# chzhang18/RAG

Hardware: AMD Instinct MI355X
Metric: disparity maps/sec at 384x1248 D=192 (Matching-Net forward) (higher is better)
Workload: dtype f32 (RAGMI_F32X3: level-3/6/12 3x3x3 convolutions with fp32 operands split into power-of-two-scaled FP16 hi+lo halves on the 16-bit matrix cores, hi*hi + hi*lo + lo*hi, fp32 accumulate: fp32-class accuracy, bound in include/rag_amd.h; strict_fp32 holds the RAGMI_F32 number); 1 GPU; BASELINE configs[1]: 1 stereo pair(s)/GPU/step, 384x1248, D=192, f32, all-conv genotype, (left_fea,right_fea)->disp, inputs resident in HBM; global_batch=1, launch=hipGraph, ranks_seen=1

## Files before the change

### rag_amd/csrc/disp.hip

```cpp
#include "disp_common.h"

namespace ragmi {

struct DispArgs {
  const void* cost;
  float* out;
  DispGeom g;
};

struct DispMoments {
  float pv = 0.f, m1 = 0.f, m2 = 0.f, xs = 0.f, pk = 0.f;
  float b1[3] = {0.f, 0.f, 0.f}, b2[3] = {0.f, 0.f, 0.f};
  __device__ __forceinline__ void add_chain(int j, float e, float x, float fd) {
    const float t = fd - pv, et = e * t;
    b1[j] += et;
    b2[j] = fmaf(et, t, b2[j]);
    xs = fmaf(e, x, xs);
    pk = fmaxf(pk, e);
  }
  __device__ __forceinline__ void flush() {
    m1 += (b1[0] + b1[1]) + b1[2];
    m2 += (b2[0] + b2[1]) + b2[2];
    b1[0] = b1[1] = b1[2] = b2[0] = b2[1] = b2[2] = 0.f;
  }
  __device__ __forceinline__ void store(float* stats, int64_t b, int64_t npix, int64_t o, float s) const {
    const float c = m1 / s;
    float* const p = stats + b * 3 * npix + o;
    p[0] = fmaxf(fmaf(-c, c, m2 / s), 0.f);
    p[npix] = pk / s;
    p[2 * npix] = fmaxf(fmaf(-0.6931471805599453f, xs / s, logf(s)), 0.f);
  }
};

struct DispWindow {
  float ks = 0.f, rf = 0.f, w0 = 0.f, w1 = 0.f;
  float c0[3] = {0.f, 0.f, 0.f}, c1[3] = {0.f, 0.f, 0.f};
  __device__ __forceinline__ void add_chain(int j, float e, float fd) {
    const float t = fd - ks, ew = fabsf(t) <= rf ? e : 0.f;
    c0[j] += ew;
    c1[j] = fmaf(ew, t, c1[j]);
  }
  __device__ __forceinline__ void flush() {
    w0 += (c0[0] + c0[1]) + c0[2];
    w1 += (c1[0] + c1[1]) + c1[2];
    c0[0] = c0[1] = c0[2] = c1[0] = c1[1] = c1[2] = 0.f;
  }
  __device__ __forceinline__ void store(float* mode, int64_t b, int64_t npix, int64_t o, float s) const {
    float* const p = mode + b * 3 * npix + o;
    p[0] = ks;
    p[npix] = w0 > 0.f ? ks + w1 / w0 : ks;
    p[2 * npix] = w0 / s;
  }
};

template <class T, bool STATS, bool MODE>
__global__ __launch_bounds__(256) void disp_softargmin_kernel(DispArgs a, float* stats, float* mode, int radius) {
  static_assert(STATS || !MODE, "the mode instantiations write the statistics too");
  extern __shared__ float4 ztab[];
  const DispGeom& g = a.g;
  disp_fill_taps(ztab, g);
  __syncthreads();
  const int64_t npix = (int64_t)g.Ho * g.Wo;
  const int64_t o = (int64_t)blockIdx.x * 256 + threadIdx.x;
  if (o >= npix) return;
  const int b = blockIdx.y;
  const DispPlaneSampler<T> smp(static_cast<const T*>(a.cost) + (int64_t)b * g.d * (g.h * g.w), g, (int)(o / g.Wo), (int)(o % g.Wo));
  DispSoftmax sm;
  DispMoments mo;
  DispWalk walk(ztab, smp, g.d);
  for (int dd = 0; dd < g.maxdisp; ++dd) {
    const float t = walk.sample(dd);
    const DispSoftmax::Step k = sm.weigh(t);
    if constexpr (STATS) {
      if (k.up) {
        mo.flush();
        const float dl = (float)dd - mo.pv;
        mo.m2 = k.x * fmaf(dl, fmaf(dl, sm.s, -2.f * mo.m1), mo.m2);
        mo.m1 = k.x * fmaf(-dl, sm.s, mo.m1);
        mo.xs = sm.s > 0.f ? k.x * fmaf(k.xa, sm.s, mo.xs) : 0.f;
        mo.pv = (float)dd;
        mo.pk = 1.f;
      } else {
        mo.add_chain(0, k.x, k.xa, (float)dd);
      }
      if ((dd & 15) == 15) mo.flush();
    }
    sm.add(k, dd, t);
  }
  const float s = sm.s;
  a.out[(int64_t)b * npix + o] = sm.ws / s;
  if constexpr (STATS) {
    mo.flush();
    mo.store(stats, b, npix, o, s);
  }
  if constexpr (MODE) {
    DispWindow wd;
    wd.ks = mo.pv;
    wd.rf = (float)radius;
    const int ks = (int)mo.pv, d_lo = max(ks - radius, 0), d_hi = min(ks + radius, g.maxdisp - 1);
    DispWalk window(ztab, smp, g.d, (int)ztab[d_lo].x);
    for (int dd = d_lo; dd <= d_hi; ++dd) {
      wd.add_chain(0, __builtin_amdgcn_exp2f((window.sample(dd) - sm.m) * DISP_LOG2E), (float)dd);
      if (((dd - d_lo) & 15) == 15) wd.flush();
    }
    wd.flush();
    wd.store(mode, b, npix, o, s);
  }
}

constexpr int DX3_TY = 8, DX3_TX = 32, DX3_CR = 5, DX3_CC = 13, DX3_CP = DX3_CR * DX3_CC;

template <class T, bool STATS, bool MODE>
__global__ __launch_bounds__(256) void disp_softargmin_x3_kernel(DispArgs a, float* stats, float* mode, int radius) {
  static_assert(STATS || !MODE, "the mode instantiations write the statistics too");
  extern __shared__ __attribute__((aligned(16))) float dx3_lds[];
  const DispGeom& g = a.g;
  float4* const ztab = reinterpret_cast<float4*>(dx3_lds);
  float* const tile = dx3_lds + 4 * g.maxdisp;
  const int tid = threadIdx.x, tx = tid % DX3_TX, ty = tid / DX3_TX;
  const int ntx = (g.Wo + DX3_TX - 1) / DX3_TX, nty = (g.Ho + DX3_TY - 1) / DX3_TY, ntile = ntx * nty;
  const int chunk = (ntile + 7) / 8, jb = blockIdx.x;
  const int tidx = (jb & 7) * chunk + (jb >> 3);
  if ((jb >> 3) >= chunk || tidx >= ntile) return;
  const int ox0 = (tidx % ntx) * DX3_TX, oy0 = (tidx / ntx) * DX3_TY, b = blockIdx.z;
  const int ox = min(ox0 + tx, g.Wo - 1), oy = min(oy0 + ty, g.Ho - 1);
  const int cy0 = lin_index(oy0, g.h, g.Ho, g.sh, 0).i0, cx0 = lin_index(ox0, g.w, g.Wo, g.sw, 0).i0;
  const int hw = g.h * g.w, D = g.d;
  const T* base = static_cast<const T*>(a.cost) + (int64_t)b * D * hw;
  for (int i = tid; i < D * DX3_CP; i += 256) {
    const int z = i / DX3_CP, r = i % DX3_CP;
    const int gy = min(cy0 + r / DX3_CC, g.h - 1), gx = min(cx0 + r % DX3_CC, g.w - 1);
    tile[i] = ld(base + (int64_t)z * hw + gy * g.w + gx);
  }
  for (int dd = tid; dd < g.maxdisp; dd += 256) {
    const LinIdx lz = lin_index(dd, D, g.maxdisp, g.sd, 0);
    const int k = dd / 3;
    float4 e = make_float4(0.f, 0.f, 0.f, (float)dd);
    if (lz.i0 < k) { e.x = lz.w0; e.y = lz.w1; }
    else if (lz.i1 != lz.i0) { e.y = lz.w0; e.z = lz.w1; }
    else e.y = lz.w0 + lz.w1;
    ztab[dd] = e;
  }
  const LinIdx ly = lin_index(oy, g.h, g.Ho, g.sh, 0);
  const LinIdx lx = lin_index(ox, g.w, g.Wo, g.sw, 0);
  const float* const t00 = tile + (ly.i0 - cy0) * DX3_CC + (lx.i0 - cx0);
  const float* const t01 = t00 + (lx.i1 - lx.i0);
  const float* const t10 = t00 + (ly.i1 - ly.i0) * DX3_CC;
  const float* const t11 = t10 + (lx.i1 - lx.i0);
  __syncthreads();
  auto plane = [&](int z) {
    const int o = z * DX3_CP;
    return lerp2(ly.w0, lerp2(lx.w0, t00[o], lx.w1, t01[o]), ly.w1, lerp2(lx.w0, t10[o], lx.w1, t11[o]));
  };
  float s = 0.f, ws = 0.f;
  DispMoments mo;
  int am = 0;
  DispWindow wd;
  wd.rf = (float)radius;
  float lo = INFINITY;
  auto sample = [&](int j, const float4 tb, float vp, float vc, float vn) __attribute__((always_inline)) {
    const float c = fmaf(tb.x, vp, fmaf(tb.y, vc, tb.z * vn));
    const float x = (lo - c) * DISP_LOG2E;
    const float e = __builtin_amdgcn_exp2f(x);
    s += e;
    ws = fmaf(e, tb.w, ws);
    if constexpr (STATS) mo.add_chain(j, e, x, tb.w);
    if constexpr (MODE) wd.add_chain(j, e, tb.w);
  };
  auto fold = [&]() __attribute__((always_inline)) {
    if constexpr (STATS) mo.flush();
    if constexpr (MODE) wd.flush();
  };
  if (D == 64) {
    float v[64];
#pragma unroll
    for (int z = 0; z < 64; ++z) {
      v[z] = plane(z);
      lo = fminf(lo, v[z]);
      if ((z & 7) == 7) __builtin_amdgcn_sched_barrier(0);
    }
    if constexpr (STATS) {
#pragma unroll
      for (int z = 63; z >= 0; --z) am = v[z] == lo ? z : am;
      mo.pv = (float)(3 * am + 1);
      if constexpr (MODE) wd.ks = am == 0 ? 0.f : mo.pv;
      __builtin_amdgcn_sched_barrier(0);
    }
#pragma unroll
    for (int k = 0; k < 64; ++k) {
      const float vp_ = v[k > 0 ? k - 1 : 0], vc_ = v[k], vn_ = v[k < 63 ? k + 1 : 63];
#pragma unroll
      for (int j = 0; j < 3; ++j) sample(j, ztab[3 * k + j], vp_, vc_, vn_);
      if ((k & 7) == 7) {
        fold();
        __builtin_amdgcn_sched_barrier(0);
      }
    }
  } else {
#pragma clang loop unroll_count(4) vectorize(disable)
  for (int z = 0; z < D; ++z) {
    const float vz = plane(z);
    if constexpr (STATS) am = vz < lo ? z : am;
    lo = fminf(lo, vz);
  }
  if constexpr (STATS) mo.pv = (float)(3 * am + 1);
  if constexpr (MODE) wd.ks = am == 0 ? 0.f : mo.pv;
  float vc = plane(0), vp = vc, vn = plane(min(1, D - 1));
  for (int k = 0; k < D; ++k) {
#pragma unroll
    for (int j = 0; j < 3; ++j) sample(j, ztab[3 * k + j], vp, vc, vn);
    vp = vc; vc = vn; vn = plane(min(k + 2, D - 1));
    if ((k & 7) == 7) fold();
  }
  fold();
  }
  if (ox0 + tx < g.Wo && oy0 + ty < g.Ho) {
    a.out[(int64_t)b * g.Ho * g.Wo + (int64_t)oy * g.Wo + ox] = ws / s;
    if constexpr (STATS) mo.store(stats, b, (int64_t)g.Ho * g.Wo, (int64_t)oy * g.Wo + ox, s);
    if constexpr (MODE) wd.store(mode, b, (int64_t)g.Ho * g.Wo, (int64_t)oy * g.Wo + ox, s);
  }
}

template <class T, bool STATS, bool MODE>
__global__ __launch_bounds__(256) void disparity_regression_kernel(const T* __restrict__ prob, float* __restrict__ out, float* __restrict__ stats,
                                                                  float* __restrict__ mode, int D, int64_t hw, int radius) {
  static_assert(STATS || !MODE, "the mode instantiations write the statistics too");
  const int64_t o = (int64_t)blockIdx.x * 256 + threadIdx.x;
  if (o >= hw) return;
  const int b = blockIdx.y;
  const T* p = prob + (int64_t)b * D * hw + o;
  float acc = 0.f;
#pragma unroll 8
  for (int dd = 0; dd < D; ++dd) acc = fmaf(ld(p + (int64_t)dd * hw), (float)dd, acc);
  out[(int64_t)b * hw + o] = acc;
  if constexpr (STATS) {
    float var[8] = {0.f, 0.f, 0.f, 0.f, 0.f, 0.f, 0.f, 0.f}, ent[8] = {0.f, 0.f, 0.f, 0.f, 0.f, 0.f, 0.f, 0.f}, pk = 0.f;
    float best = -INFINITY;
    int ks = 0;
    for (int d0 = 0; d0 < D; d0 += 8) {
      static_for<8>([&](auto J) {
        constexpr int j = decltype(J)::value;
        if (d0 + j < D) {
          const float q = ld(p + (int64_t)(d0 + j) * hw), t = (float)(d0 + j) - acc;
          var[j] = fmaf(q * t, t, var[j]);
          ent[j] = q > 0.f ? fmaf(q, logf(q), ent[j]) : ent[j];
          pk = fmaxf(pk, q);
          if constexpr (MODE) {
            if (q > best) {
              best = q;
              ks = d0 + j;
            }
          }
        }
      });
    }
    float* const st = stats + (int64_t)b * 3 * hw + o;
    st[0] = ((var[0] + var[1]) + (var[2] + var[3])) + ((var[4] + var[5]) + (var[6] + var[7]));
    st[hw] = pk;
    st[2 * hw] = 0.f - (((ent[0] + ent[1]) + (ent[2] + ent[3])) + ((ent[4] + ent[5]) + (ent[6] + ent[7])));
    if constexpr (MODE) {
      float w0[8] = {0.f, 0.f, 0.f, 0.f, 0.f, 0.f, 0.f, 0.f}, w1[8] = {0.f, 0.f, 0.f, 0.f, 0.f, 0.f, 0.f, 0.f};
      const int d_lo = max(ks - radius, 0), d_hi = min(ks + radius, D - 1);
      for (int d0 = d_lo; d0 <= d_hi; d0 += 8) {
        static_for<8>([&](auto J) {
          constexpr int j = decltype(J)::value;
          if (d0 + j <= d_hi) {
            const float q = ld(p + (int64_t)(d0 + j) * hw);
            w0[j] += q;
            w1[j] = fmaf(q, (float)(d0 + j - ks), w1[j]);
          }
        });
      }
      const float m0 = ((w0[0] + w0[1]) + (w0[2] + w0[3])) + ((w0[4] + w0[5]) + (w0[6] + w0[7]));
      const float m1 = ((w1[0] + w1[1]) + (w1[2] + w1[3])) + ((w1[4] + w1[5]) + (w1[6] + w1[7]));
      float* const mp = mode + (int64_t)b * 3 * hw + o;
      mp[0] = (float)ks;
      mp[hw] = m0 != 0.f ? (float)ks + m1 / m0 : (float)ks;
      mp[2 * hw] = m0;
    }
  }
}

template <bool STATS, bool MODE>
int launch_disp_softargmin(const char* name, const void* cost, void* out, void* stats, void* mode, int B, int d, int h, int w,
                           int maxdisp, int Ho, int Wo, int radius, int dtype, void* stream) {
  RAGMI_REQUIRE(B > 0 && d > 0 && h > 0 && w > 0 && maxdisp > 0 && Ho > 0 && Wo > 0, RAGMI_EINVAL, "%s: non-positive size", name);
  if constexpr (MODE)
    RAGMI_REQUIRE(radius >= 0 && radius <= maxdisp, RAGMI_EINVAL, "%s: radius %d not in [0, maxdisp = %d]", name, radius, maxdisp);
  RAGMI_REQUIRE(dtype_ok(dtype), RAGMI_EUNSUPPORTED, "%s: dtype %d not built", name, dtype);
  RAGMI_REQUIRE(B <= 65535 && (int64_t)h * w < (1ll << 30), RAGMI_EUNSUPPORTED, "%s: size too large", name);
  const DispArgs a{cost, (float*)out, disp_geom(d, h, w, maxdisp, Ho, Wo)};
  const size_t lds = (size_t)maxdisp * sizeof(float4);
  RAGMI_REQUIRE(lds <= 64 * 1024, RAGMI_EUNSUPPORTED, "%s: maxdisp %d exceeds the tap table (4096)", name, maxdisp);
  const size_t lds3 = lds + (size_t)d * DX3_CP * sizeof(float);
  const bool tiled = maxdisp == 3 * d && Ho == 3 * h && Wo == 3 * w && lds3 <= 64 * 1024, bf16 = dtype == RAGMI_BF16;
  const dim3 grid((unsigned)ceil_div((int64_t)Ho * Wo, 256), B);
  const dim3 g3((unsigned)ceil_div(Wo, DX3_TX), (unsigned)ceil_div(Ho, DX3_TY), (unsigned)B);
  const dim3 g1((unsigned)(ceil_div((int64_t)g3.x * g3.y, 8) * 8), 1, (unsigned)B);
  void (*const kernel)(DispArgs, float*, float*, int) =
      tiled ? (bf16 ? disp_softargmin_x3_kernel<bf16_t, STATS, MODE> : disp_softargmin_x3_kernel<float, STATS, MODE>)
            : (bf16 ? disp_softargmin_kernel<bf16_t, STATS, MODE> : disp_softargmin_kernel<float, STATS, MODE>);
  hipLaunchKernelGGL(kernel, tiled ? g1 : grid, dim3(256), tiled ? lds3 : lds, static_cast<hipStream_t>(stream), a, (float*)stats,
                     (float*)mode, radius);
  return check_launch(name);
}

template <bool STATS, bool MODE>
int launch_disparity_regression(const char* name, const void* prob, void* out, void* stats, void* mode, int B, int D, int H, int W,
                                int radius, int dtype, void* stream) {
  RAGMI_REQUIRE(B > 0 && D > 0 && H > 0 && W > 0, RAGMI_EINVAL, "%s: non-positive size", name);
  if constexpr (MODE) RAGMI_REQUIRE(radius >= 0 && radius <= D, RAGMI_EINVAL, "%s: radius %d not in [0, D = %d]", name, radius, D);
  RAGMI_REQUIRE(dtype_ok(dtype), RAGMI_EUNSUPPORTED, "%s: dtype %d not built", name, dtype);
  RAGMI_REQUIRE(B <= 65535, RAGMI_EUNSUPPORTED, "%s: B too large", name);
  const int64_t hw = (int64_t)H * W;
  const dim3 grid((unsigned)ceil_div(hw, 256), B);
  const hipStream_t q = static_cast<hipStream_t>(stream);
  if (dtype == RAGMI_BF16)
    hipLaunchKernelGGL((disparity_regression_kernel<bf16_t, STATS, MODE>), grid, dim3(256), 0, q, (const bf16_t*)prob, (float*)out,
                       (float*)stats, (float*)mode, D, hw, radius);
  else
    hipLaunchKernelGGL((disparity_regression_kernel<float, STATS, MODE>), grid, dim3(256), 0, q, (const float*)prob, (float*)out,
                       (float*)stats, (float*)mode, D, hw, radius);
  return check_launch(name);
}

}

extern "C" int ragmi_disp_softargmin_fwd(const void* cost, void* out, int B, int d, int h, int w, int maxdisp, int Ho,
                                         int Wo, int dtype, void* stream) {
  RAGMI_REQUIRE(cost && out, RAGMI_EINVAL, "disp_softargmin: null pointer");
  return ragmi::launch_disp_softargmin<false, false>("disp_softargmin", cost, out, nullptr, nullptr, B, d, h, w, maxdisp, Ho, Wo, 0, dtype,
                                                     stream);
}
extern "C" int ragmi_disp_softargmin_stats_fwd(const void* cost, void* out, void* stats, int B, int d, int h, int w, int maxdisp,
                                               int Ho, int Wo, int dtype, void* stream) {
  RAGMI_REQUIRE(cost && out && stats, RAGMI_EINVAL, "disp_softargmin_stats: null pointer");
  return ragmi::launch_disp_softargmin<true, false>("disp_softargmin_stats", cost, out, stats, nullptr, B, d, h, w, maxdisp, Ho, Wo, 0,
                                                    dtype, stream);
}
extern "C" int ragmi_disp_softargmin_mode_fwd(const void* cost, void* out, void* stats, void* mode, int B, int d, int h, int w,
                                              int maxdisp, int Ho, int Wo, int radius, int dtype, void* stream) {
  RAGMI_REQUIRE(cost && out && stats && mode, RAGMI_EINVAL, "disp_softargmin_mode: null pointer");
  return ragmi::launch_disp_softargmin<true, true>("disp_softargmin_mode", cost, out, stats, mode, B, d, h, w, maxdisp, Ho, Wo, radius,
                                                   dtype, stream);
}

extern "C" int ragmi_disparity_regression_fwd(const void* prob, void* out, int B, int D, int H, int W, int dtype,
                                              void* stream) {
  RAGMI_REQUIRE(prob && out, RAGMI_EINVAL, "disparity_regression: null pointer");
  return ragmi::launch_disparity_regression<false, false>("disparity_regression", prob, out, nullptr, nullptr, B, D, H, W, 0, dtype, stream);
}
extern "C" int ragmi_disparity_regression_stats_fwd(const void* prob, void* out, void* stats, int B, int D, int H, int W, int dtype,
                                                    void* stream) {
  RAGMI_REQUIRE(prob && out && stats, RAGMI_EINVAL, "disparity_regression_stats: null pointer");
  return ragmi::launch_disparity_regression<true, false>("disparity_regression_stats", prob, out, stats, nullptr, B, D, H, W, 0, dtype,
                                                         stream);
}
extern "C" int ragmi_disparity_regression_mode_fwd(const void* prob, void* out, void* stats, void* mode, int B, int D, int H, int W,
                                                   int radius, int dtype, void* stream) {
  RAGMI_REQUIRE(prob && out && stats && mode, RAGMI_EINVAL, "disparity_regression_mode: null pointer");
  return ragmi::launch_disparity_regression<true, true>("disparity_regression_mode", prob, out, stats, mode, B, D, H, W, radius, dtype,
                                                        stream);
}
```

### rag_amd/csrc/disp_common.h

```cpp
#pragma once
#include "common.h"

namespace ragmi {

struct DispGeom {
  int d, h, w, maxdisp, Ho, Wo;
  float sd, sh, sw;
};
inline DispGeom disp_geom(int d, int h, int w, int maxdisp, int Ho, int Wo) {
  return DispGeom{d, h, w, maxdisp, Ho, Wo, lin_scale(d, maxdisp, 0), lin_scale(h, Ho, 0), lin_scale(w, Wo, 0)};
}

constexpr float DISP_LOG2E = 1.4426950408889634f;

__device__ __forceinline__ void disp_fill_taps(float4* ztab, const DispGeom& g) {
  for (int dd = threadIdx.x; dd < g.maxdisp; dd += 256) {
    const LinIdx lz = lin_index(dd, g.d, g.maxdisp, g.sd, 0);
    const bool same = lz.i1 == lz.i0;
    ztab[dd] = make_float4((float)lz.i0, lz.w0, same ? 0.f : lz.w1, same ? lz.w1 : 0.f);
  }
}

template <class T>
struct DispPlaneSampler {
  const T* base;
  int hw, o00, o01, o10, o11;
  float wy0, wy1, wx0, wx1;
  __device__ __forceinline__ DispPlaneSampler(const T* cost, const DispGeom& g, int oy, int ox) : base(cost), hw(g.h * g.w) {
    const LinIdx ly = lin_index(oy, g.h, g.Ho, g.sh, 0);
    const LinIdx lx = lin_index(ox, g.w, g.Wo, g.sw, 0);
    o00 = ly.i0 * g.w + lx.i0, o01 = ly.i0 * g.w + lx.i1;
    o10 = ly.i1 * g.w + lx.i0, o11 = ly.i1 * g.w + lx.i1;
    wy0 = ly.w0, wy1 = ly.w1, wx0 = lx.w0, wx1 = lx.w1;
  }
  __device__ __forceinline__ float plane(int z) const {
    const T* p = base + (int64_t)z * hw;
    return lerp2(wy0, lerp2(wx0, ld(p + o00), wx1, ld(p + o01)), wy1, lerp2(wx0, ld(p + o10), wx1, ld(p + o11)));
  }
};

template <class Sampler>
struct DispWalk {
  const float4* ztab;
  const Sampler& smp;
  int d, cz;
  float b0, b1;
  __device__ __forceinline__ DispWalk(const float4* taps, const Sampler& sampler, int planes, int cz0 = 0)
      : ztab(taps), smp(sampler), d(planes), cz(cz0), b0(sampler.plane(cz0)), b1(sampler.plane(cz0 + 1 < planes ? cz0 + 1 : planes - 1)) {}
  __device__ __forceinline__ float sample(int dd) {
    const float4 tb = ztab[dd];
    const int i0 = (int)tb.x;
    while (i0 > cz) {
      ++cz;
      b0 = b1;
      b1 = smp.plane(cz + 1 < d ? cz + 1 : d - 1);
    }
    return -fmaf(tb.y + tb.w, b0, tb.z * b1);
  }
};

struct DispSoftmax {
  float m = -INFINITY, s = 0.f, ws = 0.f;
  struct Step {
    bool up;
    float x, xa;
  };
  __device__ __forceinline__ Step weigh(float t) const {
    const bool up = t > m;
    const float xa = (up ? m - t : t - m) * DISP_LOG2E;
    return Step{up, __builtin_amdgcn_exp2f(xa), xa};
  }
  __device__ __forceinline__ void add(const Step& k, int dd, float t) {
    const float r = k.up ? k.x : 1.f, e = k.up ? 1.f : k.x;
    s = fmaf(s, r, e);
    ws = fmaf(ws, r, e * (float)dd);
    m = k.up ? t : m;
  }
};

constexpr int DISP_BWD_T = 16, DISP_BWD_WIN = 8;

}
```

Baseline: 1209 disparity maps/s.

## Factor softargmin exponentials into per-plane cube roots, dropping the tap table

```diff
diff --git a/rag_amd/csrc/disp.hip b/rag_amd/csrc/disp.hip
--- a/rag_amd/csrc/disp.hip
+++ b/rag_amd/csrc/disp.hip
@@ -115,8 +115,7 @@
   static_assert(STATS || !MODE, "the mode instantiations write the statistics too");
   extern __shared__ __attribute__((aligned(16))) float dx3_lds[];
   const DispGeom& g = a.g;
-  float4* const ztab = reinterpret_cast<float4*>(dx3_lds);
-  float* const tile = dx3_lds + 4 * g.maxdisp;
+  float* const tile = dx3_lds;
   const int tid = threadIdx.x, tx = tid % DX3_TX, ty = tid / DX3_TX;
   const int ntx = (g.Wo + DX3_TX - 1) / DX3_TX, nty = (g.Ho + DX3_TY - 1) / DX3_TY, ntile = ntx * nty;
   const int chunk = (ntile + 7) / 8, jb = blockIdx.x;
@@ -131,15 +130,6 @@
     const int z = i / DX3_CP, r = i % DX3_CP;
     const int gy = min(cy0 + r / DX3_CC, g.h - 1), gx = min(cx0 + r % DX3_CC, g.w - 1);
     tile[i] = ld(base + (int64_t)z * hw + gy * g.w + gx);
-  }
-  for (int dd = tid; dd < g.maxdisp; dd += 256) {
-    const LinIdx lz = lin_index(dd, D, g.maxdisp, g.sd, 0);
-    const int k = dd / 3;
-    float4 e = make_float4(0.f, 0.f, 0.f, (float)dd);
-    if (lz.i0 < k) { e.x = lz.w0; e.y = lz.w1; }
-    else if (lz.i1 != lz.i0) { e.y = lz.w0; e.z = lz.w1; }
-    else e.y = lz.w0 + lz.w1;
-    ztab[dd] = e;
   }
   const LinIdx ly = lin_index(oy, g.h, g.Ho, g.sh, 0);
   const LinIdx lx = lin_index(ox, g.w, g.Wo, g.sw, 0);
@@ -158,14 +148,17 @@
   DispWindow wd;
   wd.rf = (float)radius;
   float lo = INFINITY;
-  auto sample = [&](int j, const float4 tb, float vp, float vc, float vn) __attribute__((always_inline)) {
-    const float c = fmaf(tb.x, vp, fmaf(tb.y, vc, tb.z * vn));
-    const float x = (lo - c) * DISP_LOG2E;
-    const float e = __builtin_amdgcn_exp2f(x);
-    s += e;
-    ws = fmaf(e, tb.w, ws);
-    if constexpr (STATS) mo.add_chain(j, e, x, tb.w);
-    if constexpr (MODE) wd.add_chain(j, e, tb.w);
+  auto third = [&](float vz) __attribute__((always_inline)) { return (lo - vz) * DISP_LOG2E_3; };
+  auto samples = [&](float fd0, float cp, float cc, float cn, float xp, float xc, float xn) __attribute__((always_inline)) {
+    const DispThirds t(cp, cc, cn, xp, xc, xn);
+#pragma unroll
+    for (int j = 0; j < 3; ++j) {
+      const float fd = fd0 + (float)j;
+      s += t.e[j];
+      ws = fmaf(t.e[j], fd, ws);
+      if constexpr (STATS) mo.add_chain(j, t.e[j], t.x[j], fd);
+      if constexpr (MODE) wd.add_chain(j, t.e[j], fd);
+    }
   };
   auto fold = [&]() __attribute__((always_inline)) {
     if constexpr (STATS) mo.flush();
@@ -186,11 +179,12 @@
       if constexpr (MODE) wd.ks = am == 0 ? 0.f : mo.pv;
       __builtin_amdgcn_sched_barrier(0);
     }
+    float xc = third(v[0]), cc = __builtin_amdgcn_exp2f(xc), xp = xc, cp = cc;
 #pragma unroll
     for (int k = 0; k < 64; ++k) {
-      const float vp_ = v[k > 0 ? k - 1 : 0], vc_ = v[k], vn_ = v[k < 63 ? k + 1 : 63];
-#pragma unroll
-      for (int j = 0; j < 3; ++j) sample(j, ztab[3 * k + j], vp_, vc_, vn_);
+      const float xn = k < 63 ? third(v[(k + 1) & 63]) : xc, cn = k < 63 ? __builtin_amdgcn_exp2f(xn) : cc;
+      samples((float)(3 * k), cp, cc, cn, xp, xc, xn);
+      xp = xc, cp = cc, xc = xn, cc = cn;
       if ((k & 7) == 7) {
         fold();
         __builtin_amdgcn_sched_barrier(0);
@@ -205,11 +199,11 @@
   }
   if constexpr (STATS) mo.pv = (float)(3 * am + 1);
   if constexpr (MODE) wd.ks = am == 0 ? 0.f : mo.pv;
-  float vc = plane(0), vp = vc, vn = plane(min(1, D - 1));
+  float xc = third(plane(0)), cc = __builtin_amdgcn_exp2f(xc), xp = xc, cp = cc, fd0 = 0.f;
   for (int k = 0; k < D; ++k) {
-#pragma unroll
-    for (int j = 0; j < 3; ++j) sample(j, ztab[3 * k + j], vp, vc, vn);
-    vp = vc; vc = vn; vn = plane(min(k + 2, D - 1));
+    const float xn = third(plane(min(k + 1, D - 1))), cn = __builtin_amdgcn_exp2f(xn);
+    samples(fd0, cp, cc, cn, xp, xc, xn);
+    xp = xc, cp = cc, xc = xn, cc = cn, fd0 += 3.f;
     if ((k & 7) == 7) fold();
   }
   fold();
@@ -292,8 +286,8 @@
   const DispArgs a{cost, (float*)out, disp_geom(d, h, w, maxdisp, Ho, Wo)};
   const size_t lds = (size_t)maxdisp * sizeof(float4);
   RAGMI_REQUIRE(lds <= 64 * 1024, RAGMI_EUNSUPPORTED, "%s: maxdisp %d exceeds the tap table (4096)", name, maxdisp);
-  const size_t lds3 = lds + (size_t)d * DX3_CP * sizeof(float);
-  const bool tiled = maxdisp == 3 * d && Ho == 3 * h && Wo == 3 * w && lds3 <= 64 * 1024, bf16 = dtype == RAGMI_BF16;
+  const size_t lds3 = (size_t)d * DX3_CP * sizeof(float);
+  const bool tiled = maxdisp == 3 * d && Ho == 3 * h && Wo == 3 * w && lds + lds3 <= 64 * 1024, bf16 = dtype == RAGMI_BF16;
   const dim3 grid((unsigned)ceil_div((int64_t)Ho * Wo, 256), B);
   const dim3 g3((unsigned)ceil_div(Wo, DX3_TX), (unsigned)ceil_div(Ho, DX3_TY), (unsigned)B);
   const dim3 g1((unsigned)(ceil_div((int64_t)g3.x * g3.y, 8) * 8), 1, (unsigned)B);
diff --git a/rag_amd/csrc/disp_common.h b/rag_amd/csrc/disp_common.h
--- a/rag_amd/csrc/disp_common.h
+++ b/rag_amd/csrc/disp_common.h
@@ -12,6 +12,17 @@
 }
 
 constexpr float DISP_LOG2E = 1.4426950408889634f;
+
+constexpr float DISP_LOG2E_3 = 0.48089834696298783f;
+struct DispThirds {
+  float e[3], x[3];
+  __device__ __forceinline__ DispThirds(float cp, float cc, float cn, float xp, float xc, float xn) {
+#pragma clang fp contract(off)
+    const float q = cc * cc;
+    e[0] = q * cp, e[1] = q * cc, e[2] = q * cn;
+    x[0] = fmaf(2.f, xc, xp), x[1] = 3.f * xc, x[2] = fmaf(2.f, xc, xn);
+  }
+};
 
 __device__ __forceinline__ void disp_fill_taps(float4* ztab, const DispGeom& g) {
   for (int dd = threadIdx.x; dd < g.maxdisp; dd += 256) {
```

Measured after the change: 1218 disparity maps/s (median of 6 runs). Within noise of the previous version (+0.8%).
